# kyle-wedgwood/ArmadilloCUDALinearInterpolation

Hardware: AMD Instinct MI355X
Metric: interpolated points/sec (fp64) (higher is better)
Workload: dtype f64

## Files before the change

armadillocudalinearinterpolation_amd/csrc/mi_interp1.hip:

```cpp
#include <algorithm>
#include <cmath>
#include <cstdlib>

#include "mi_interp1_stream.hpp"
#include "mi_interp1_sweep.hpp"

using namespace mi_interp1;

namespace {

struct SweepEnv {
    long min_bytes;
    size_t min_tiles_per_cu;
    int variant;
    bool variant_forced;
};
const SweepEnv& sweep_env()
{
    static const SweepEnv e = [] {
        SweepEnv v{-1, kSweepMinTilesPerCu, 2, false};
        if (const char* s = getenv("MI_SWEEP_MIN_BYTES")) v.min_bytes = (long)strtoull(s, nullptr, 10);
        if (const char* s = getenv("MI_SWEEP_MIN_TILES_PER_CU")) v.min_tiles_per_cu = (size_t)strtoull(s, nullptr, 10);
        if (const char* s = getenv("MI_SWEEP_VARIANT")) {
            const int x = atoi(s);
            v.variant = (x == 1 || x == 2) ? x : 2;
            v.variant_forced = true;
        }
        return v;
    }();
    return e;
}

constexpr int kGatedBlock = 256, kGatedVpl = 2;
template <int MODE, int FORMULA, int BLOCK, int VPL>
mi_status launch_vec_shape(mi_ctx* ctx, const G1Dev& d, const double* xq, double* yq, size_t nq, double extrap,
                           const int* order_flag, const ProbeArgs& probe)
{
    const size_t lanes = (nq >> 1) + (nq & 1);
    const size_t per_block = (size_t)BLOCK * VPL;
    const size_t grid = (lanes + per_block - 1) / per_block;
    if (grid > 0x7fffffffull) return mi::fail(ctx, MI_ERR_INVALID_ARG, "mi_interp1_f64_dev: nq=%zu too large for one launch", nq);
    hipLaunchKernelGGL((interp1_vec_kernel<MODE, FORMULA, BLOCK, VPL>), dim3((unsigned)grid), dim3(BLOCK), 0, ctx->stream,
                       d, xq, yq, nq, extrap, order_flag, probe);
    MI_LAUNCH_CHECK(ctx, "interp1 streaming kernel");
    return MI_OK;
}

template <int MODE, int FORMULA>
mi_status launch_vec(mi_ctx* ctx, const G1Dev& d, const double* xq, double* yq, size_t nq, double extrap,
                     const int* order_flag = nullptr, const ProbeArgs& probe = ProbeArgs{})
{
    if (order_flag)
        return launch_vec_shape<MODE, FORMULA, kGatedBlock, kGatedVpl>(ctx, d, xq, yq, nq, extrap, order_flag, probe);
    return launch_vec_shape<MODE, FORMULA, kBlock, kVecVpl>(ctx, d, xq, yq, nq, extrap, nullptr, probe);
}

template <int MODE, int FORMULA = 0>
mi_status launch_mode(mi_ctx* ctx, const G1Dev& d, size_t table_bytes, const double* xq, double* yq, size_t nq,
                      double extrap)
{
    const bool aligned = ((reinterpret_cast<uintptr_t>(xq) | reinterpret_cast<uintptr_t>(yq)) & 15u) == 0;
    if (!aligned) {
        const size_t grid = (nq + kBlock - 1) / kBlock;
        if (grid > 0x7fffffffull) return mi::fail(ctx, MI_ERR_INVALID_ARG, "mi_interp1_f64_dev: nq=%zu too large for one launch", nq);
        hipLaunchKernelGGL((interp1_scalar_kernel<MODE, FORMULA>), dim3((unsigned)grid), dim3(kBlock), 0, ctx->stream, d, xq, yq,
                           nq, extrap);
        MI_LAUNCH_CHECK(ctx, "interp1 scalar kernel");
        return MI_OK;
    }
    const unsigned cus = (unsigned)(ctx->compute_units > 0 ? ctx->compute_units : 256);
    const size_t ntiles = nq / kSweepTile;
    bool size_ok = table_bytes >= ((size_t)5 << 20);
    if (MODE == 3) size_ok = table_bytes > kLdsMaxTableBytes && !(table_bytes > 2600000 && table_bytes < 3900000);
    if (sweep_env().min_bytes >= 0) size_ok = table_bytes >= (size_t)sweep_env().min_bytes;
    const bool sweep_ok = ctx->query_order != MI_QUERIES_ORDERED && size_ok &&
                          ntiles >= (size_t)cus * sweep_env().min_tiles_per_cu && std::isfinite(d.xmax - d.xmin) && (d.xmax - d.xmin) > 0.0;
    if constexpr (MODE == 0 || MODE == 3) {
        const size_t ybytes = ((size_t)d.n + 1) * (MODE == 0 ? sizeof(double) : sizeof(d2));
        if (ctx->query_order != MI_QUERIES_ORDERED && ybytes > (MODE == 0 ? kLdsMinTableBytes0 : kLdsMinTableBytes3) && ybytes <= kLdsMaxTableBytes &&
            nq >= 8 * kLdsQueriesPerBlock && std::isfinite(d.xmax - d.xmin) && (d.xmax - d.xmin) > 0.0) {
            ProbeArgs probe{};
            if (ctx->query_order == MI_QUERIES_AUTO) {
                const int predicted = *reinterpret_cast<volatile int*>(ctx->probe_host);
                probe = ProbeArgs{xq, nq, d.xmin, (double)kSweepBins / (d.xmax - d.xmin), nullptr, ctx->probe_host_dev};
                if (predicted == 1) return launch_vec<MODE, FORMULA>(ctx, d, xq, yq, nq, extrap, nullptr, probe);
            }
            MI_HIP(ctx, hipFuncSetAttribute(reinterpret_cast<const void*>(&interp1_lds_kernel<MODE, FORMULA>),
                                            hipFuncAttributeMaxDynamicSharedMemorySize, (int)kLdsMaxTableBytes));
            const size_t grid = (nq + kLdsQueriesPerBlock - 1) / kLdsQueriesPerBlock;
            hipLaunchKernelGGL((interp1_lds_kernel<MODE, FORMULA>), dim3((unsigned)grid), dim3(kLdsBlock), ybytes, ctx->stream, d, xq,
                               yq, nq, extrap, probe);
            MI_LAUNCH_CHECK(ctx, "interp1 LDS-table kernel");
            return MI_OK;
        }
    }
    if (!sweep_ok) return launch_vec<MODE, FORMULA>(ctx, d, xq, yq, nq, extrap);

    const double bscale = (double)kSweepBins / (d.xmax - d.xmin);
    int* flags = reinterpret_cast<int*>(static_cast<char*>(ctx->reduce_ws) + mi_ctx::kFlagOffset);
    const size_t head = ntiles * kSweepTile;
    const unsigned grid = (unsigned)std::min<size_t>(ntiles, (size_t)cus);
    int plan = 0;
    ProbeArgs probe{};
    if (ctx->query_order == MI_QUERIES_AUTO) {
        const int predicted = *reinterpret_cast<volatile int*>(ctx->probe_host);
        plan = (predicted == 0 || predicted == 1) ? predicted : 2;
        probe = ProbeArgs{xq, nq, d.xmin, bscale, plan == 2 ? flags + 2 : nullptr, ctx->probe_host_dev};
    }
    if (plan == 1) return launch_vec<MODE, FORMULA>(ctx, d, xq, yq, nq, extrap, nullptr, probe);
    if (plan == 2) {
        hipLaunchKernelGGL(interp1_order_probe, dim3(1), dim3(64), 0, ctx->stream, probe);
        MI_LAUNCH_CHECK(ctx, "interp1 order probe");
        hipLaunchKernelGGL((interp1_sweep_kernel<MODE, FORMULA>), dim3(grid), dim3(kSweepThreads), 0, ctx->stream, d, xq,
                           yq, ntiles, extrap, bscale, flags + 2, (size_t)0, ProbeArgs{});
        MI_LAUNCH_CHECK(ctx, "interp1 region-sweep kernel");
        mi_status st = launch_vec<MODE, FORMULA>(ctx, d, xq, yq, head, extrap, flags + 2);
        if (st != MI_OK) return st;
        if (nq > head) return launch_vec<MODE, FORMULA>(ctx, d, xq + head, yq + head, nq - head, extrap);
        return MI_OK;
    }
    if (sweep_env().variant == 2 && (sweep_env().variant_forced || ntiles >= (size_t)cus * 16)) {
        const unsigned pgrid = (unsigned)std::min<size_t>(ntiles, (size_t)cus);
        hipLaunchKernelGGL((interp1_sweep_pipe_kernel<MODE, FORMULA>), dim3(pgrid), dim3(kPipeThreads), 0, ctx->stream, d, xq, yq,
                           ntiles, extrap, bscale, flags, nq - head, probe);
        MI_LAUNCH_CHECK(ctx, "interp1 pipelined region-sweep kernel");
        return MI_OK;
    }
    hipLaunchKernelGGL((interp1_sweep_kernel<MODE, FORMULA>), dim3(grid), dim3(kSweepThreads), 0, ctx->stream, d, xq, yq,
                       ntiles, extrap, bscale, flags, nq - head, probe);
    MI_LAUNCH_CHECK(ctx, "interp1 region-sweep kernel");
    return MI_OK;
}

}

extern "C" {

mi_status mi_interp1_f64_dev(mi_ctx* ctx, const mi_grid1* g, const double* xq, double* yq, size_t nq, double extrap)
{
    MI_REQUIRE(ctx, ctx && g, "mi_interp1_f64_dev: NULL context or grid");
    if (nq == 0) return MI_OK;
    MI_REQUIRE(ctx, xq && yq, "mi_interp1_f64_dev: NULL query/result pointer");
    MI_REQUIRE(ctx, ((reinterpret_cast<uintptr_t>(xq) | reinterpret_cast<uintptr_t>(yq)) & 7u) == 0,
               "mi_interp1_f64_dev: pointers must be 8-byte aligned");
    MI_HIP(ctx, hipSetDevice(ctx->device));
    switch (g->mode) {
        case 0:
            if (g->d.formula == 1) return launch_mode<0, 1>(ctx, g->d, g->table_bytes, xq, yq, nq, extrap);
            if (g->d.formula == 2) return launch_mode<0, 2>(ctx, g->d, g->table_bytes, xq, yq, nq, extrap);
            if (g->d.formula == 3) return launch_mode<0, 3>(ctx, g->d, g->table_bytes, xq, yq, nq, extrap);
            return launch_mode<0, 0>(ctx, g->d, g->table_bytes, xq, yq, nq, extrap);
        case 1:
            if (g->d.centred) return launch_mode<3>(ctx, g->d, g->table_bytes, xq, yq, nq, extrap);
            return launch_mode<1>(ctx, g->d, g->table_bytes, xq, yq, nq, extrap);
        default: return launch_mode<2>(ctx, g->d, g->table_bytes, xq, yq, nq, extrap);
    }
}

mi_status mi_interp1_f64_host(mi_ctx* ctx, const mi_grid1* g, const double* xq, double* yq, size_t nq, double extrap)
{
    MI_REQUIRE(ctx, ctx && g, "mi_interp1_f64_host: NULL context or grid");
    if (nq == 0) return MI_OK;
    MI_REQUIRE(ctx, xq && yq, "mi_interp1_f64_host: NULL query/result pointer");
    MI_HIP(ctx, hipSetDevice(ctx->device));
    const size_t bytes = nq * sizeof(double);
    mi_status st = mi::ensure_scratch(ctx, 0, bytes);
    if (st != MI_OK) return st;
    st = mi::ensure_scratch(ctx, 1, bytes);
    if (st != MI_OK) return st;
    const size_t chunk = (size_t)8 << 20;
    if (nq <= 2 * chunk) {
        MI_HIP(ctx, hipMemcpyAsync(ctx->scratch[0], xq, bytes, hipMemcpyHostToDevice, ctx->stream));
        st = mi_interp1_f64_dev(ctx, g, (const double*)ctx->scratch[0], (double*)ctx->scratch[1], nq, extrap);
        if (st != MI_OK) return st;
        MI_HIP(ctx, hipMemcpyAsync(yq, ctx->scratch[1], bytes, hipMemcpyDeviceToHost, ctx->stream));
        MI_HIP(ctx, hipStreamSynchronize(ctx->stream));
        return MI_OK;
    }
    st = mi::ensure_aux_stream(ctx);
    if (st != MI_OK) return st;
    const bool pin_in = mi::pin_host(xq, bytes), pin_out = mi::pin_host(yq, bytes);
    const double* din = (const double*)ctx->scratch[0];
    double* dout = (double*)ctx->scratch[1];
    hipError_t herr = hipSuccess;
    const char* what = "";
    if (getenv("MI_TEST_FAIL_HOST_CHUNK")) { herr = hipErrorUnknown; what = "MI_TEST_FAIL_HOST_CHUNK (error-path test hook)"; }
    for (size_t off = 0; off < nq && herr == hipSuccess && st == MI_OK; off += chunk) {
        const size_t m = std::min(chunk, nq - off);
        herr = hipMemcpyAsync((void*)(din + off), xq + off, m * sizeof(double), hipMemcpyHostToDevice, ctx->stream);
        if (herr != hipSuccess) { what = "upload of a query chunk"; break; }
        st = mi_interp1_f64_dev(ctx, g, din + off, dout + off, m, extrap);
        if (st != MI_OK) break;
        herr = hipEventRecord(ctx->aux_event, ctx->stream);
        if (herr == hipSuccess) herr = hipStreamWaitEvent(ctx->aux_stream, ctx->aux_event, 0);
        if (herr == hipSuccess) herr = hipMemcpyAsync(yq + off, dout + off, m * sizeof(double), hipMemcpyDeviceToHost, ctx->aux_stream);
        if (herr != hipSuccess) what = "download of a result chunk";
    }
    const hipError_t e1 = hipStreamSynchronize(ctx->stream), e2 = hipStreamSynchronize(ctx->aux_stream);
    if (pin_in) mi::unpin_host(xq);
    if (pin_out) mi::unpin_host(yq);
    if (st != MI_OK) return st;
    if (herr != hipSuccess) return mi::fail(ctx, MI_ERR_HIP, "mi_interp1_f64_host: %s failed: %s", what, hipGetErrorString(herr));
    MI_HIP(ctx, e1);
    MI_HIP(ctx, e2);
    return MI_OK;
}

mi_status mi_interp1_f64(mi_ctx* ctx, const double* x, const double* y, size_t n, const double* xq, double* yq,
                         size_t nq, double extrap)
{
    mi_grid1* g = nullptr;
    mi_status st = mi_grid1_create(ctx, x, y, n, MI_GRID_SANITISE, &g);
    if (st != MI_OK) return st;
    st = mi_interp1_f64_host(ctx, g, xq, yq, nq, extrap);
    mi_grid1_destroy(g);
    return st;
}

}
```

armadillocudalinearinterpolation_amd/csrc/mi_interp1_sweep.hpp:

```cpp
#pragma once
#include "mi_interp1_eval.hpp"

namespace mi_interp1 {

__device__ __forceinline__ d2 stream_load(const d2* p) { return __builtin_nontemporal_load(p); }
__device__ __forceinline__ void stream_store(d2 v, d2* p) { __builtin_nontemporal_store(v, p); }

constexpr size_t kSweepMinTilesPerCu = 2;
constexpr int kSweepM3Batch = 4;
constexpr bool kSweepWin = false;
constexpr int kSweepThreads = 512;
constexpr int kSweepK = 32;
constexpr int kSweepTile = kSweepThreads * kSweepK;
template <int MODE, int FORMULA>
__global__ __launch_bounds__(kSweepThreads) void interp1_sweep_kernel(G1Dev g, const double* __restrict__ xq,
                                                                      double* __restrict__ yq, size_t ntiles,
                                                                      double extrap, double bscale,
                                                                      const int* __restrict__ order_flag,
                                                                      size_t tail, ProbeArgs probe)
{
    __shared__ double sq[kSweepTile];
    __shared__ unsigned hist[kSweepBins];
    const int tid = threadIdx.x;
    if (*order_flag != 0) return;
    const bool last_wg = blockIdx.x == gridDim.x - 1;
    if (probe.host_mailbox && last_wg && tid < 64) order_probe_wave(probe);
    bool rev = false;
    for (size_t t = blockIdx.x; t < ntiles; t += gridDim.x, rev = !rev) {
        const d2* q2 = reinterpret_cast<const d2*>(xq + t * kSweepTile);
        d2* o2 = reinterpret_cast<d2*>(yq + t * kSweepTile);
        double q[kSweepK];
#pragma unroll
        for (int u = 0; u < kSweepK / 2; ++u) {
            const d2 v = stream_load(q2 + tid + u * kSweepThreads);
            q[2 * u] = v.x;
            q[2 * u + 1] = v.y;
        }
        for (int b = tid; b < kSweepBins; b += kSweepThreads) hist[b] = 0;
        __syncthreads();
        unsigned short bin[kSweepK], rank[kSweepK];
#pragma unroll
        for (int u = 0; u < kSweepK; ++u) {
            const int b = sweep_bin(q[u], g.xmin, bscale);
            bin[u] = (unsigned short)b;
            rank[u] = (unsigned short)atomicAdd(&hist[b], 1u);
        }
        __syncthreads();
        if (tid < 64) {
            unsigned run = 0;
#pragma unroll
            for (int base = 0; base < kSweepBins; base += 64) {
                const unsigned v = hist[base + tid];
                unsigned incl = v;
#pragma unroll
                for (int off = 1; off < 64; off <<= 1) {
                    const unsigned o = __shfl_up(incl, off, 64);
                    if (tid >= off) incl += o;
                }
                hist[base + tid] = run + incl - v;
                run += __shfl(incl, 63, 64);
            }
        }
        __syncthreads();
        unsigned short sp[kSweepK];
#pragma unroll
        for (int u = 0; u < kSweepK; ++u) {
            sp[u] = (unsigned short)(hist[bin[u]] + rank[u]);
            sq[sp[u]] = q[u];
        }
        __syncthreads();
#pragma unroll
        for (int u = 0; u < kSweepK; u += 4) {
            double qq[4], rr[4];
#pragma unroll
            for (int w = 0; w < 4; ++w) {
                const int p = tid + (u + w) * kSweepThreads;
                qq[w] = sq[rev ? kSweepTile - 1 - p : p];
            }
            eval_batch<MODE, 4, FORMULA, kSweepWin>(g, qq, rr, extrap);
#pragma unroll
            for (int w = 0; w < 4; ++w) {
                const int p = tid + (u + w) * kSweepThreads;
                sq[rev ? kSweepTile - 1 - p : p] = rr[w];
            }
        }
        __syncthreads();
#pragma unroll
        for (int u = 0; u < kSweepK / 2; ++u) {
            d2 v;
            v.x = sq[sp[2 * u]];
            v.y = sq[sp[2 * u + 1]];
            stream_store(v, o2 + tid + u * kSweepThreads);
        }
        __syncthreads();
    }
    if (tail && last_wg) {
        const double* tq = xq + ntiles * kSweepTile;
        double* to = yq + ntiles * kSweepTile;
        double q[kSweepK];
#pragma unroll
        for (int u = 0; u < kSweepK; ++u) {
            const size_t i = (size_t)tid + (size_t)u * kSweepThreads;
            q[u] = i < tail ? tq[i] : 0.0;
        }
#pragma unroll
        for (int u = 0; u < kSweepK; u += 4) {
            const double qq[4] = {q[u], q[u + 1], q[u + 2], q[u + 3]};
            double rr[4];
            eval_batch<MODE, 4, FORMULA, kSweepWin>(g, qq, rr, extrap);
#pragma unroll
            for (int w = 0; w < 4; ++w) {
                const size_t i = (size_t)tid + (size_t)(u + w) * kSweepThreads;
                if (i < tail) to[i] = rr[w];
            }
        }
    }
}

constexpr int kPipeGroup = 512;
constexpr int kPipeThreads = 2 * kPipeGroup;
static_assert(kSweepTile == kPipeGroup * kSweepK, "one group covers a tile with kSweepK queries per lane");

__device__ __forceinline__ void pipe_barrier()
{
    asm volatile("s_waitcnt lgkmcnt(0)\n\ts_barrier" ::: "memory");
}

template <int MODE, int FORMULA>
__device__ __forceinline__ void pipe_gather_rounds(const G1Dev& g, double* sq, int first, int stride, double extrap)
{
    constexpr int B = (MODE == 3) ? kSweepM3Batch : 4;
#pragma unroll 1
    for (int r = 0; r < 8 / B; ++r) {
        double qq[B], rr[B];
#pragma unroll
        for (int w = 0; w < B; ++w) qq[w] = sq[first + (B * r + w) * stride];
        eval_batch<MODE, B, FORMULA, kSweepWin>(g, qq, rr, extrap);
#pragma unroll
        for (int w = 0; w < B; ++w) sq[first + (B * r + w) * stride] = rr[w];
    }
}

template <int MODE, int FORMULA>
__global__ __launch_bounds__(kPipeThreads) void interp1_sweep_pipe_kernel(G1Dev g, const double* __restrict__ xq,
                                                                          double* __restrict__ yq, size_t ntiles,
                                                                          double extrap, double bscale,
                                                                          const int* __restrict__ order_flag,
                                                                          size_t tail, ProbeArgs probe)
{
    __shared__ double sq[kSweepTile];
    __shared__ unsigned hist[2][kSweepBins];
    __shared__ unsigned gbar[2];
    if (*order_flag != 0) return;
    if (threadIdx.x < 2) gbar[threadIdx.x] = 0;
    const int tid = threadIdx.x & (kPipeGroup - 1);
    const int grp = threadIdx.x >> 9;
    const bool last_wg = blockIdx.x == gridDim.x - 1;
    if (probe.host_mailbox && last_wg && threadIdx.x >= kPipeThreads - 64) order_probe_wave(probe);
    const long nloc = ntiles > blockIdx.x ? (long)((ntiles - blockIdx.x + gridDim.x - 1) / gridDim.x) : 0;
    double q[kSweepK];
    unsigned sp2[kSweepK / 2];
    auto load_tile = [&](long it) {
        const d2* q2 = reinterpret_cast<const d2*>(xq + ((size_t)blockIdx.x + (size_t)it * gridDim.x) * kSweepTile);
#pragma unroll
        for (int u = 0; u < kSweepK / 2; ++u) {
            const d2 v = stream_load(q2 + tid + u * kPipeGroup);
            q[2 * u] = v.x;
            q[2 * u + 1] = v.y;
        }
    };
    auto store_tile = [&](long it) {
        d2* o2 = reinterpret_cast<d2*>(yq + ((size_t)blockIdx.x + (size_t)it * gridDim.x) * kSweepTile);
#pragma unroll
        for (int u = 0; u < kSweepK / 2; ++u) {
            d2 v;
            v.x = q[2 * u];
            v.y = q[2 * u + 1];
            stream_store(v, o2 + tid + u * kPipeGroup);
        }
    };
    for (int b = threadIdx.x; b < 2 * kSweepBins; b += kPipeThreads) (&hist[0][0])[b] = 0;
    if (grp == 0 && nloc > 0) load_tile(0);
    pipe_barrier();
    unsigned* const myhist = hist[grp];
    unsigned gb_target = 0;
    auto group_barrier = [&]() {
        gb_target += kPipeGroup / 64;
        asm volatile("s_waitcnt lgkmcnt(0)" ::: "memory");
        if ((threadIdx.x & 63) == 0) atomicAdd(&gbar[grp], 1u);
        while (*reinterpret_cast<volatile unsigned*>(&gbar[grp]) < gb_target) __builtin_amdgcn_s_sleep(2);
        asm volatile("" ::: "memory");
    };
    auto gather_step = [&](long it) {
        const bool act = it >= 0;
        const bool rev = (it & 1) != 0;
        const int stride = rev ? -kPipeGroup : kPipeGroup;
        int first = rev ? kSweepTile - 1 - tid : tid;
        if (act) {
#pragma unroll 1
            for (int iv = 0; iv < 4; ++iv) {
                pipe_gather_rounds<MODE, FORMULA>(g, sq, first, stride, extrap);
                first += 8 * stride;
            }
        }
        pipe_barrier();
        if (act) {
#pragma unroll
            for (int u = 0; u < kSweepK; u += 2) {
                q[u] = sq[sp2[u / 2] & 0xffffu];
                q[u + 1] = sq[sp2[u / 2] >> 16];
                if ((u & 6) == 6) __builtin_amdgcn_sched_barrier(0);
            }
        } else {
#pragma unroll
            for (int u = 0; u < kSweepK; ++u) q[u] = 0.0;
        }
        pipe_barrier();
        if (act) store_tile(it);
        if (it + 2 < nloc) {
            load_tile(it + 2);
        } else {
#pragma unroll
            for (int u = 0; u < kSweepK; ++u) q[u] = 0.0;
        }
        pipe_barrier();
    };
    auto prep_step = [&](long it) {
        const bool act = it + 1 < nloc;
        unsigned rank2[kSweepK / 2];
#pragma unroll
        for (int u = 0; u < kSweepK / 2; ++u) rank2[u] = 0;
        if (act) {
#pragma unroll
            for (int u = 0; u < kSweepK; u += 2) {
                const unsigned r0 = atomicAdd(&myhist[sweep_bin(q[u], g.xmin, bscale)], 1u);
                const unsigned r1 = atomicAdd(&myhist[sweep_bin(q[u + 1], g.xmin, bscale)], 1u);
                rank2[u / 2] = r0 | (r1 << 16);
                if ((u & 6) == 6) __builtin_amdgcn_sched_barrier(0);
            }
            group_barrier();
            if (tid < 64) {
                unsigned run = 0;
#pragma unroll
                for (int base = 0; base < kSweepBins; base += 64) {
                    const unsigned v = myhist[base + tid];
                    unsigned incl = v;
#pragma unroll
                    for (int off = 1; off < 64; off <<= 1) {
                        const unsigned o = __shfl_up(incl, off, 64);
                        if (tid >= off) incl += o;
                    }
                    myhist[base + tid] = run + incl - v;
                    run += __shfl(incl, 63, 64);
                }
            }
            group_barrier();
#pragma unroll
            for (int u = 0; u < kSweepK; u += 2) {
                double qa = q[u], qb = q[u + 1];
                asm volatile("" : "+v"(qa), "+v"(qb));
                const unsigned p0 = myhist[sweep_bin(qa, g.xmin, bscale)] + (rank2[u / 2] & 0xffffu);
                const unsigned p1 = myhist[sweep_bin(qb, g.xmin, bscale)] + (rank2[u / 2] >> 16);
                sp2[u / 2] = p0 | (p1 << 16);
                if ((u & 6) == 6) __builtin_amdgcn_sched_barrier(0);
            }
        } else {
#pragma unroll
            for (int u = 0; u < kSweepK / 2; ++u) sp2[u] = 0;
        }
        pipe_barrier();
        if (act) {
            for (int b = tid; b < kSweepBins; b += kPipeGroup) myhist[b] = 0;
        }
        pipe_barrier();
        if (act) {
#pragma unroll
            for (int u = 0; u < kSweepK; u += 2) {
                sq[sp2[u / 2] & 0xffffu] = q[u];
                sq[sp2[u / 2] >> 16] = q[u + 1];
                if ((u & 6) == 6) __builtin_amdgcn_sched_barrier(0);
            }
        }
        pipe_barrier();
    };
    if (grp == 0) {
        for (long it = -1;;) {
            prep_step(it);
            if (++it >= nloc) break;
            gather_step(it);
            if (++it >= nloc) break;
        }
    } else {
        for (long it = -1;;) {
            gather_step(it);
            if (++it >= nloc) break;
            prep_step(it);
            if (++it >= nloc) break;
        }
    }
    if (tail && last_wg && grp == 0) {
        const double* tq = xq + ntiles * kSweepTile;
        double* to = yq + ntiles * kSweepTile;
#pragma unroll 1
        for (int u = 0; u < kSweepK; u += 4) {
            double qq[4], rr[4];
#pragma unroll
            for (int w = 0; w < 4; ++w) {
                const size_t i = (size_t)tid + (size_t)(u + w) * kPipeGroup;
                qq[w] = i < tail ? tq[i] : 0.0;
            }
            eval_batch<MODE, 4, FORMULA, kSweepWin>(g, qq, rr, extrap);
#pragma unroll
            for (int w = 0; w < 4; ++w) {
                const size_t i = (size_t)tid + (size_t)(u + w) * kPipeGroup;
                if (i < tail) to[i] = rr[w];
            }
        }
    }
}

}
```

Baseline: 151.0 billion.

## Partition queries into contiguous per-workgroup ranges with variable-size pipelined tiles

The pipelined sweep kernel now gives each workgroup one contiguous range of query pairs. The range is split into a few tiles of up to 39 pairs per lane, replacing the fixed 16K-query tiles interleaved across workgroups, and the separate single-workgroup tail is dropped. The aim is to balance work across CUs, cut the number of pipeline iterations and barriers, and remove the serialized tail, with gather raised in wave priority via s_setprio. In exchange there are more registers per lane (40 doubles), more LDS, and per-element bounds predicates in every loop.

```diff
diff --git a/armadillocudalinearinterpolation_amd/csrc/mi_interp1.hip b/armadillocudalinearinterpolation_amd/csrc/mi_interp1.hip
--- a/armadillocudalinearinterpolation_amd/csrc/mi_interp1.hip
+++ b/armadillocudalinearinterpolation_amd/csrc/mi_interp1.hip
@@ -120,9 +120,8 @@
         return MI_OK;
     }
     if (sweep_env().variant == 2 && (sweep_env().variant_forced || ntiles >= (size_t)cus * 16)) {
-        const unsigned pgrid = (unsigned)std::min<size_t>(ntiles, (size_t)cus);
-        hipLaunchKernelGGL((interp1_sweep_pipe_kernel<MODE, FORMULA>), dim3(pgrid), dim3(kPipeThreads), 0, ctx->stream, d, xq, yq,
-                           ntiles, extrap, bscale, flags, nq - head, probe);
+        hipLaunchKernelGGL((interp1_sweep_pipe_kernel<MODE, FORMULA>), dim3(cus), dim3(kPipeThreads), 0, ctx->stream, d, xq, yq,
+                           nq, extrap, bscale, flags, probe);
         MI_LAUNCH_CHECK(ctx, "interp1 pipelined region-sweep kernel");
         return MI_OK;
     }
diff --git a/armadillocudalinearinterpolation_amd/csrc/mi_interp1_sweep.hpp b/armadillocudalinearinterpolation_amd/csrc/mi_interp1_sweep.hpp
--- a/armadillocudalinearinterpolation_amd/csrc/mi_interp1_sweep.hpp
+++ b/armadillocudalinearinterpolation_amd/csrc/mi_interp1_sweep.hpp
@@ -119,7 +119,10 @@
 
 constexpr int kPipeGroup = 512;
 constexpr int kPipeThreads = 2 * kPipeGroup;
-static_assert(kSweepTile == kPipeGroup * kSweepK, "one group covers a tile with kSweepK queries per lane");
+constexpr int kPipeVecs = 20;
+constexpr int kPipeTileMax = kPipeGroup * 39;
+static_assert(kPipeTileMax <= 2 * kPipeVecs * kPipeGroup, "a group's registers hold the largest tile");
+static_assert(kPipeTileMax % 2 == 0 && kPipeTileMax < 65536, "whole pairs; sorted positions are 16-bit");
 
 __device__ __forceinline__ void pipe_barrier()
 {
@@ -127,28 +130,37 @@
 }
 
 template <int MODE, int FORMULA>
-__device__ __forceinline__ void pipe_gather_rounds(const G1Dev& g, double* sq, int first, int stride, double extrap)
+__device__ __forceinline__ void pipe_gather_rounds(const G1Dev& g, double* sq, int len, int first, int stride, double extrap)
 {
     constexpr int B = (MODE == 3) ? kSweepM3Batch : 4;
+    const int tid = threadIdx.x & (kPipeGroup - 1);
+    const int wbase = __builtin_amdgcn_readfirstlane(tid) & ~63;
+    const int nb = len > wbase ? (len - wbase + B * kPipeGroup - 1) / (B * kPipeGroup) : 0;
+    const int edge = stride > 0 ? len - 1 : 0;
 #pragma unroll 1
-    for (int r = 0; r < 8 / B; ++r) {
+    for (int r = 0; r < nb; ++r) {
         double qq[B], rr[B];
-#pragma unroll
-        for (int w = 0; w < B; ++w) qq[w] = sq[first + (B * r + w) * stride];
+        int p[B];
+#pragma unroll
+        for (int w = 0; w < B; ++w) {
+            p[w] = tid + (B * r + w) * kPipeGroup < len ? first + (B * r + w) * stride : -1;
+            qq[w] = sq[p[w] >= 0 ? p[w] : edge];
+        }
         eval_batch<MODE, B, FORMULA, kSweepWin>(g, qq, rr, extrap);
 #pragma unroll
-        for (int w = 0; w < B; ++w) sq[first + (B * r + w) * stride] = rr[w];
+        for (int w = 0; w < B; ++w)
+            if (p[w] >= 0) sq[p[w]] = rr[w];
     }
 }
 
 template <int MODE, int FORMULA>
 __global__ __launch_bounds__(kPipeThreads) void interp1_sweep_pipe_kernel(G1Dev g, const double* __restrict__ xq,
-                                                                          double* __restrict__ yq, size_t ntiles,
+                                                                          double* __restrict__ yq, size_t nq,
                                                                           double extrap, double bscale,
                                                                           const int* __restrict__ order_flag,
-                                                                          size_t tail, ProbeArgs probe)
+                                                                          ProbeArgs probe)
 {
-    __shared__ double sq[kSweepTile];
+    __shared__ double sq[kPipeTileMax];
     __shared__ unsigned hist[2][kSweepBins];
     __shared__ unsigned gbar[2];
     if (*order_flag != 0) return;
@@ -157,26 +169,40 @@
     const int grp = threadIdx.x >> 9;
     const bool last_wg = blockIdx.x == gridDim.x - 1;
     if (probe.host_mailbox && last_wg && threadIdx.x >= kPipeThreads - 64) order_probe_wave(probe);
-    const long nloc = ntiles > blockIdx.x ? (long)((ntiles - blockIdx.x + gridDim.x - 1) / gridDim.x) : 0;
-    double q[kSweepK];
-    unsigned sp2[kSweepK / 2];
-    auto load_tile = [&](long it) {
-        const d2* q2 = reinterpret_cast<const d2*>(xq + ((size_t)blockIdx.x + (size_t)it * gridDim.x) * kSweepTile);
-#pragma unroll
-        for (int u = 0; u < kSweepK / 2; ++u) {
-            const d2 v = stream_load(q2 + tid + u * kPipeGroup);
+    const size_t npairs = nq >> 1, per_wg = npairs / gridDim.x, extra_wg = npairs % gridDim.x;
+    const size_t range_first = (size_t)blockIdx.x * per_wg + min((size_t)blockIdx.x, extra_wg);
+    const size_t range_pairs = per_wg + (blockIdx.x < extra_wg ? 1 : 0);
+    const int nloc = (int)((2 * (per_wg + (extra_wg ? 1 : 0)) + kPipeTileMax - 1) / kPipeTileMax);
+    const int per_tile = nloc > 0 ? (int)(range_pairs / (size_t)nloc) : 0, extra_tile = nloc > 0 ? (int)(range_pairs % (size_t)nloc) : 0;
+    auto tile_pairs = [&](int it) { return per_tile + (it < extra_tile ? 1 : 0); };
+    auto tile_first = [&](int it) { return range_first + (size_t)it * (size_t)per_tile + (size_t)min(it, extra_tile); };
+    auto avail = [&](int pairs) {
+        int a = pairs - tid;
+        asm volatile("" : "+v"(a));
+        return a;
+    };
+    double q[2 * kPipeVecs];
+    unsigned sp2[kPipeVecs];
+    auto load_tile = [&](int it) {
+        const d2* q2 = reinterpret_cast<const d2*>(xq) + tile_first(it) + tid;
+        const int av = avail(tile_pairs(it));
+#pragma unroll
+        for (int u = 0; u < kPipeVecs; ++u) {
+            d2 v = {0.0, 0.0};
+            if (u * kPipeGroup < av) v = stream_load(q2 + u * kPipeGroup);
             q[2 * u] = v.x;
             q[2 * u + 1] = v.y;
         }
     };
-    auto store_tile = [&](long it) {
-        d2* o2 = reinterpret_cast<d2*>(yq + ((size_t)blockIdx.x + (size_t)it * gridDim.x) * kSweepTile);
-#pragma unroll
-        for (int u = 0; u < kSweepK / 2; ++u) {
+    auto store_tile = [&](int it) {
+        d2* o2 = reinterpret_cast<d2*>(yq) + tile_first(it) + tid;
+        const int av = avail(tile_pairs(it));
+#pragma unroll
+        for (int u = 0; u < kPipeVecs; ++u) {
             d2 v;
             v.x = q[2 * u];
             v.y = q[2 * u + 1];
-            stream_store(v, o2 + tid + u * kPipeGroup);
+            if (u * kPipeGroup < av) stream_store(v, o2 + u * kPipeGroup);
         }
     };
     for (int b = threadIdx.x; b < 2 * kSweepBins; b += kPipeThreads) (&hist[0][0])[b] = 0;
@@ -191,29 +217,26 @@
         while (*reinterpret_cast<volatile unsigned*>(&gbar[grp]) < gb_target) __builtin_amdgcn_s_sleep(2);
         asm volatile("" ::: "memory");
     };
-    auto gather_step = [&](long it) {
+    auto gather_step = [&](int it) {
         const bool act = it >= 0;
-        const bool rev = (it & 1) != 0;
-        const int stride = rev ? -kPipeGroup : kPipeGroup;
-        int first = rev ? kSweepTile - 1 - tid : tid;
+        const int len = act ? 2 * tile_pairs(it) : 0;
         if (act) {
-#pragma unroll 1
-            for (int iv = 0; iv < 4; ++iv) {
-                pipe_gather_rounds<MODE, FORMULA>(g, sq, first, stride, extrap);
-                first += 8 * stride;
-            }
-        }
-        pipe_barrier();
-        if (act) {
-#pragma unroll
-            for (int u = 0; u < kSweepK; u += 2) {
+            const bool rev = (it & 1) != 0;
+            __builtin_amdgcn_s_setprio(3);
+            pipe_gather_rounds<MODE, FORMULA>(g, sq, len, rev ? len - 1 - tid : tid, rev ? -kPipeGroup : kPipeGroup, extrap);
+            __builtin_amdgcn_s_setprio(0);
+        }
+        pipe_barrier();
+        const int av = avail(len / 2);
+#pragma unroll
+        for (int u = 0; u < 2 * kPipeVecs; u += 2) {
+            q[u] = 0.0;
+            q[u + 1] = 0.0;
+            if (u / 2 * kPipeGroup < av) {
                 q[u] = sq[sp2[u / 2] & 0xffffu];
                 q[u + 1] = sq[sp2[u / 2] >> 16];
-                if ((u & 6) == 6) __builtin_amdgcn_sched_barrier(0);
-            }
-        } else {
-#pragma unroll
-            for (int u = 0; u < kSweepK; ++u) q[u] = 0.0;
+            }
+            if ((u & 6) == 6) __builtin_amdgcn_sched_barrier(0);
         }
         pipe_barrier();
         if (act) store_tile(it);
@@ -221,21 +244,25 @@
             load_tile(it + 2);
         } else {
 #pragma unroll
-            for (int u = 0; u < kSweepK; ++u) q[u] = 0.0;
-        }
-        pipe_barrier();
-    };
-    auto prep_step = [&](long it) {
+            for (int u = 0; u < 2 * kPipeVecs; ++u) q[u] = 0.0;
+        }
+        pipe_barrier();
+    };
+    auto prep_step = [&](int it) {
         const bool act = it + 1 < nloc;
-        unsigned rank2[kSweepK / 2];
-#pragma unroll
-        for (int u = 0; u < kSweepK / 2; ++u) rank2[u] = 0;
+        const int pairs = act ? tile_pairs(it + 1) : 0;
+        unsigned rank2[kPipeVecs];
+#pragma unroll
+        for (int u = 0; u < kPipeVecs; ++u) rank2[u] = 0;
         if (act) {
-#pragma unroll
-            for (int u = 0; u < kSweepK; u += 2) {
-                const unsigned r0 = atomicAdd(&myhist[sweep_bin(q[u], g.xmin, bscale)], 1u);
-                const unsigned r1 = atomicAdd(&myhist[sweep_bin(q[u + 1], g.xmin, bscale)], 1u);
-                rank2[u / 2] = r0 | (r1 << 16);
+            const int av = avail(pairs);
+#pragma unroll
+            for (int u = 0; u < 2 * kPipeVecs; u += 2) {
+                if (u / 2 * kPipeGroup < av) {
+                    const unsigned r0 = atomicAdd(&myhist[sweep_bin(q[u], g.xmin, bscale)], 1u);
+                    const unsigned r1 = atomicAdd(&myhist[sweep_bin(q[u + 1], g.xmin, bscale)], 1u);
+                    rank2[u / 2] = r0 | (r1 << 16);
+                }
                 if ((u & 6) == 6) __builtin_amdgcn_sched_barrier(0);
             }
             group_barrier();
@@ -255,18 +282,22 @@
                 }
             }
             group_barrier();
-#pragma unroll
-            for (int u = 0; u < kSweepK; u += 2) {
+            const int av2 = avail(pairs);
+#pragma unroll
+            for (int u = 0; u < 2 * kPipeVecs; u += 2) {
                 double qa = q[u], qb = q[u + 1];
                 asm volatile("" : "+v"(qa), "+v"(qb));
-                const unsigned p0 = myhist[sweep_bin(qa, g.xmin, bscale)] + (rank2[u / 2] & 0xffffu);
-                const unsigned p1 = myhist[sweep_bin(qb, g.xmin, bscale)] + (rank2[u / 2] >> 16);
-                sp2[u / 2] = p0 | (p1 << 16);
+                sp2[u / 2] = 0;
+                if (u / 2 * kPipeGroup < av2) {
+                    const unsigned p0 = myhist[sweep_bin(qa, g.xmin, bscale)] + (rank2[u / 2] & 0xffffu);
+                    const unsigned p1 = myhist[sweep_bin(qb, g.xmin, bscale)] + (rank2[u / 2] >> 16);
+                    sp2[u / 2] = p0 | (p1 << 16);
+                }
                 if ((u & 6) == 6) __builtin_amdgcn_sched_barrier(0);
             }
         } else {
 #pragma unroll
-            for (int u = 0; u < kSweepK / 2; ++u) sp2[u] = 0;
+            for (int u = 0; u < kPipeVecs; ++u) sp2[u] = 0;
         }
         pipe_barrier();
         if (act) {
@@ -274,49 +305,39 @@
         }
         pipe_barrier();
         if (act) {
-#pragma unroll
-            for (int u = 0; u < kSweepK; u += 2) {
-                sq[sp2[u / 2] & 0xffffu] = q[u];
-                sq[sp2[u / 2] >> 16] = q[u + 1];
+            const int av = avail(pairs);
+#pragma unroll
+            for (int u = 0; u < 2 * kPipeVecs; u += 2) {
+                if (u / 2 * kPipeGroup < av) {
+                    sq[sp2[u / 2] & 0xffffu] = q[u];
+                    sq[sp2[u / 2] >> 16] = q[u + 1];
+                }
                 if ((u & 6) == 6) __builtin_amdgcn_sched_barrier(0);
             }
         }
         pipe_barrier();
     };
     if (grp == 0) {
-        for (long it = -1;;) {
+        for (int it = -1;;) {
             prep_step(it);
             if (++it >= nloc) break;
             gather_step(it);
             if (++it >= nloc) break;
         }
     } else {
-        for (long it = -1;;) {
+        for (int it = -1;;) {
             gather_step(it);
             if (++it >= nloc) break;
             prep_step(it);
             if (++it >= nloc) break;
         }
     }
-    if (tail && last_wg && grp == 0) {
-        const double* tq = xq + ntiles * kSweepTile;
-        double* to = yq + ntiles * kSweepTile;
-#pragma unroll 1
-        for (int u = 0; u < kSweepK; u += 4) {
-            double qq[4], rr[4];
-#pragma unroll
-            for (int w = 0; w < 4; ++w) {
-                const size_t i = (size_t)tid + (size_t)(u + w) * kPipeGroup;
-                qq[w] = i < tail ? tq[i] : 0.0;
-            }
-            eval_batch<MODE, 4, FORMULA, kSweepWin>(g, qq, rr, extrap);
-#pragma unroll
-            for (int w = 0; w < 4; ++w) {
-                const size_t i = (size_t)tid + (size_t)(u + w) * kPipeGroup;
-                if (i < tail) to[i] = rr[w];
-            }
-        }
-    }
-}
-
-}
+    if ((nq & 1) && last_wg && threadIdx.x == 0) {
+        const double qq[1] = {xq[nq - 1]};
+        double rr[1];
+        eval_batch<MODE, 1, FORMULA, kSweepWin>(g, qq, rr, extrap);
+        yq[nq - 1] = rr[0];
+    }
+}
+
+}
```

Result: no change. 149.8 billion (median of 2 runs) (-0.8%).
